# 12334zq/optical-flow-1

Measured on AMD Instinct MI355X. Metric: Mpix*warp-iters/s, TV-L1 1920x1080 5-scale, higher is better.
Workload: dtype f64; 1 GPU; tvl1flow 1920x1080 pair (synthetic P1), nscales=5 warps=5 tau=0.25 lambda=0.15 theta=0.3 zfactor=0.5 epsilon=0.01; one pair per step per GPU; workload_name=1080p, arithmetic_mode=tolerance, pairs_per_gpu=1040, pairs_in_flight_per_gpu=64, lockstep_group=16, streams_per_gpu=4, distinct_pairs=8

## Files before the change

optical-flow-1_amd/csrc/ofx_device.h:

```cpp
#pragma once

#include <hip/hip_runtime.h>

#define OFX_DEV __device__ __forceinline__

OFX_DEV double  ldw(const double *p) { return *p; }
OFX_DEV double  ldw(const float *p)  { return (double) *p; }
struct OfxRgb8 { unsigned char r, g, b; };
OFX_DEV unsigned gray8(unsigned r, unsigned g, unsigned b) { return (unsigned) (unsigned char) (.299 * r + .587 * g + .114 * b); }
OFX_DEV double  ldw(const unsigned char *p)  { return (double) *p; }
OFX_DEV double  ldw(const unsigned short *p) { return (double) *p; }
OFX_DEV double  ldw(const OfxRgb8 *p) { return (double) gray8(p->r, p->g, p->b); }
OFX_DEV double2 ldw2(const double2 *p) { return *p; }
OFX_DEV double2 ldw2(const float2 *p)  { float2 v = *p; return make_double2((double) v.x, (double) v.y); }
OFX_DEV double4 ldw4(const double4 *p) { return *p; }
OFX_DEV double4 ldw4(const float4 *p)
{
    float4 v = *p;
    return make_double4((double) v.x, (double) v.y, (double) v.z, (double) v.w);
}
OFX_DEV void stn(double *p, double v) { *p = v; }
OFX_DEV void stn(float *p, double v)  { *p = (float) v; }
OFX_DEV void stn2(double2 *p, double2 v) { *p = v; }
OFX_DEV void stn2(float2 *p, double2 v)  { *p = make_float2((float) v.x, (float) v.y); }
// ... 134 lines not shown
    const double r = __builtin_fma(-h, g, 0.5);
    g = __builtin_fma(g, r, g);
    double d = __builtin_fma(-g, g, x);
    h = __builtin_fma(h, r, h);
    g = __builtin_fma(d, h, g);
    d = __builtin_fma(-g, g, x);
    return __builtin_fma(d, h, g);
}
OFX_DEV double rcp_newton(double d)
{
    double r = __builtin_amdgcn_rcp(d);
    double e = __builtin_fma(-d, r, 1.0);
    r = __builtin_fma(r, e, r);
    e = __builtin_fma(-d, r, 1.0);
    return __builtin_fma(r, e, r);
}
OFX_DEV double div_unscaled(double n, double d)
{
    double r = __builtin_amdgcn_rcp(d);
    double e = __builtin_fma(-d, r, 1.0);
    r = __builtin_fma(r, e, r);
    e = __builtin_fma(-d, r, 1.0);
    r = __builtin_fma(r, e, r);
    const double q = n * r;
    const double rem = __builtin_fma(-d, q, n);
    return __builtin_fma(rem, r, q);
}
OFX_DEV double hypot_kernel_common(double ax, double ay)
{
    double h = sqrt_unscaled(ax * ax + ay * ay);
    double t1, t2;
    if (h <= 2.0 * ay) {
        const double delta = h - ay;
        t1 = ax * (2.0 * delta - ax);
        t2 = (delta - 2.0 * (ax - ay)) * delta;
    } else {
        const double delta = h - ax;
        t1 = 2.0 * delta * (ax - 2.0 * ay);
        t2 = (4.0 * delta - ay) * ay + delta * delta;
    }
    h -= div_unscaled(t1 + t2, 2.0 * h);
    return h;
}

OFX_DEV double hypot_ref(double x, double y)
{
    x = fabs(x);
    y = fabs(y);
    const double ax = x < y ? y : x;
    const double ay = x < y ? x : y;
    const double SCALE = 0x1p-600, LARGE = 0x1p+511, TINY = 0x1p-459, EPS = 0x1p-54;
#ifndef OFX_HYPOT_GENERAL_ONLY
    if (ax <= LARGE && ay >= 0x1p-383) {
        if (ax >= ay / EPS) return ax + ay;
        return hypot_kernel_common(ax, ay);
    }
#endif
    if (ax > LARGE) {
        if (ay <= ax * EPS) return ax + ay;
        return hypot_kernel(ax * SCALE, ay * SCALE) / SCALE;
    }
    if (ay < TINY) {
        if (ax >= ay / EPS) return ax + ay;
        return hypot_kernel(ax / SCALE, ay / SCALE) * SCALE;
    }
    if (ax >= ay / EPS) return ax + ay;
    return hypot_kernel(ax, ay);
}

struct BicubicTaps {
    int    col[4];
    int    row[4];
    double fx, fy;
    bool   out;
};

OFX_DEV int bc_clamp(int x, int n, bool &out)
{
    if (x < 0)  { out = true; return 0; }
    if (x >= n) { out = true; return n - 1; }
    return x;
}

OFX_DEV BicubicTaps bicubic_taps(double uu, double vv, int nx, int ny)
{
    BicubicTaps t;
    const int sx = (uu < 0) ? -1 : 1;
    const int sy = (vv < 0) ? -1 : 1;
    const int iu = (int) uu, iv = (int) vv;
    bool out = false;
    t.col[1] = bc_clamp(iu, nx, out);
    t.row[1] = bc_clamp(iv, ny, out);
    t.col[0] = bc_clamp(iu - sx, nx, out);
    t.row[0] = bc_clamp(iv - sx, ny, out);
    t.col[2] = bc_clamp(iu + sx, nx, out);
    t.row[2] = bc_clamp(iv + sy, ny, out);
    t.col[3] = bc_clamp(iu + 2 * sx, nx, out);
    t.row[3] = bc_clamp(iv + 2 * sy, ny, out);
    t.out = out;
    t.fx = uu - t.col[1];
    t.fy = vv - t.row[1];
    return t;
}

OFX_DEV double cubic_cell(double v0, double v1, double v2, double v3, double x)
{
    return v1 + 0.5 * x * (v2 - v0 + x * (2.0 * v0 - 5.0 * v1 + 4.0 * v2 - v3 + x * (3.0 * (v1 - v2) + v3 - v0)));
}

template <typename T>
OFX_DEV double bicubic_sample(const T *in, const BicubicTaps &t, int nx)
{
    double c[4];
#pragma unroll
    for (int k = 0; k < 4; k++) {
        const double v0 = ldw(in + (size_t) t.row[0] * nx + t.col[k]);
        const double v1 = ldw(in + (size_t) t.row[1] * nx + t.col[k]);
        const double v2 = ldw(in + (size_t) t.row[2] * nx + t.col[k]);
        const double v3 = ldw(in + (size_t) t.row[3] * nx + t.col[k]);
        c[k] = cubic_cell(v0, v1, v2, v3, t.fy);
    }
    return cubic_cell(c[0], c[1], c[2], c[3], t.fx);
}

template <typename V2, typename S>
OFX_DEV void bicubic_sample3(const V2 *__restrict__ pa, const S *__restrict__ pb, const BicubicTaps &t, int nx,
                             double &o0, double &o1, double &o2)
{
    const unsigned E = sizeof(S);
    const unsigned r0 = (unsigned) t.row[0] * nx * E, r1 = (unsigned) t.row[1] * nx * E;
    const unsigned r2 = (unsigned) t.row[2] * nx * E, r3 = (unsigned) t.row[3] * nx * E;
    double c0[4], c1[4], c2[4];
#pragma unroll
    for (int k = 0; k < 4; k++) {
        const unsigned ck = (unsigned) t.col[k] * E;
        const char *ba = reinterpret_cast<const char *>(pa), *bb = reinterpret_cast<const char *>(pb);
        const double2 a0 = ldw2(reinterpret_cast<const V2 *>(ba + 2 * (r0 + ck)));
        const double2 a1 = ldw2(reinterpret_cast<const V2 *>(ba + 2 * (r1 + ck)));
        const double2 a2 = ldw2(reinterpret_cast<const V2 *>(ba + 2 * (r2 + ck)));
        const double2 a3 = ldw2(reinterpret_cast<const V2 *>(ba + 2 * (r3 + ck)));
        const double b0 = ldw(reinterpret_cast<const S *>(bb + r0 + ck));
        const double b1 = ldw(reinterpret_cast<const S *>(bb + r1 + ck));
        const double b2 = ldw(reinterpret_cast<const S *>(bb + r2 + ck));
        const double b3 = ldw(reinterpret_cast<const S *>(bb + r3 + ck));
        c0[k] = cubic_cell(a0.x, a1.x, a2.x, a3.x, t.fy);
        c1[k] = cubic_cell(a0.y, a1.y, a2.y, a3.y, t.fy);
        c2[k] = cubic_cell(b0, b1, b2, b3, t.fy);
    }
    o0 = cubic_cell(c0[0], c0[1], c0[2], c0[3], t.fx);
    o1 = cubic_cell(c1[0], c1[1], c1[2], c1[3], t.fx);
    o2 = cubic_cell(c2[0], c2[1], c2[2], c2[3], t.fx);
}

OFX_DEV double div_backward(double ac, double al, double bc, double bu, bool lef, bool rig, bool top, bool bot)
{
    if (!lef && !rig) {
        const double dxv = ac - al;
        return top ? dxv + bc : (bot ? dxv - bu : dxv + (bc - bu));
    }
    if (lef) return top ? ac + bc : (bot ? ac - bu : ac + bc - bu);
    return top ? -al + bc : (bot ? -al - bu : -al + bc - bu);
}
```

optical-flow-1_amd/csrc/ofx_tvl1.hip:

```cpp
#include "ofx_ops.h"
#include "ofx_device.h"
#include "ofx_loop.h"
#include "ofx_pairs.h"

#include <chrono>
#include <cmath>
#include <type_traits>

#define TVL1_GRAD_IS_ZERO 1E-10
#define TVL1_PRESMOOTHING_SIGMA 0.8
#define STRIP_OUT 62

#ifdef OFX_NO_RFL
#define OFX_WAVE_UNIFORM(x) (x)
#else
#define OFX_WAVE_UNIFORM(x) __builtin_amdgcn_readfirstlane(x)
#endif
template <typename T> struct RowIn {
    double2 u, p1, p2, a;
    double r;
};

template <typename V> OFX_DEV const V *at(const V *base, unsigned byte_off)
{
// ... 782 lines not shown
            if (niter > max_iter - k0) niter = max_iter - k0;
            if (scribe) dev->cursor[(launch + 1) & 1][g] = k0 + niter;
        }
    }
    if (idle) return;
    const int step = check ? 1 : 0;
    if (N == 4 && niter >= 4) {
        if constexpr (N == 4)
            tvl1_iter3_march<T, NT, STRICT, 4, N>(Uin, P1in, P2in, A, R, hu.out, h1.out, h2.out, err, slot0, step, gw, nx, ny, y0, yend,
                                                  ys, yl, lef, rig, owner, off, so, up12, up22, cur, l_t, theta, taut, ring);
    } else if (niter >= 3)
        tvl1_iter3_march<T, NT, STRICT, 3, N>(Uin, P1in, P2in, A, R, hu.out, h1.out, h2.out, err, slot0, step, gw, nx, ny, y0, yend, ys,
                                              yl, lef, rig, owner, off, so, up12, up22, cur, l_t, theta, taut);
    else if (niter == 2)
        tvl1_iter3_march<T, NT, STRICT, 2, N>(Uin, P1in, P2in, A, R, hu.out, h1.out, h2.out, err, slot0, step, gw, nx, ny, y0, yend, ys,
                                              yl, lef, rig, owner, off, so, up12, up22, cur, l_t, theta, taut);
    else
        tvl1_iter3_march<T, NT, STRICT, 1, N>(Uin, P1in, P2in, A, R, hu.out, h1.out, h2.out, err, slot0, step, gw, nx, ny, y0, yend, ys,
                                              yl, lef, rig, owner, off, so, up12, up22, cur, l_t, theta, taut);
}

template <typename T, bool NT, bool STRICT>
__global__ __launch_bounds__(256) __attribute__((amdgpu_waves_per_eu(OFX_ITER3_WAVES, OFX_ITER3_WAVES))) void k_tvl1_iter3(
    Tri<typename Pix<T>::v2> Ut, Tri<typename Pix<T>::v2> P1t, Tri<typename Pix<T>::v2> P2t,
    const typename Pix<T>::v2 *__restrict__ Ag, const T *__restrict__ Rg, double *__restrict__ errg, int k0, int check, int slot0,
    int nx, int ny, int rows, int strips_x, int strips_pad, double l_t, double theta, double taut, double eps2, unsigned incode,
    unsigned runmask, unsigned long long nit, int err_stride, OfxLoopDev *dev, int launch, double afac1, double afac2, double afac3,
    int max_iter)
{
    tvl1_unit<T, NT, STRICT, 3>(Ut, P1t, P2t, Ag, Rg, errg, k0, check, slot0, nx, ny, rows, strips_x, strips_pad, l_t, theta, taut, eps2,
                                incode, runmask, nit, err_stride, dev, launch, afac1, afac2, afac3, max_iter, nullptr);
}

template <typename T, bool NT, bool STRICT>
__global__ __launch_bounds__(256) __attribute__((amdgpu_waves_per_eu(OFX_ITER3_WAVES, OFX_ITER3_WAVES))) void k_tvl1_iter4(
    Tri<typename Pix<T>::v2> Ut, Tri<typename Pix<T>::v2> P1t, Tri<typename Pix<T>::v2> P2t,
    const typename Pix<T>::v2 *__restrict__ Ag, const T *__restrict__ Rg, double *__restrict__ errg, int k0, int check, int slot0,
    int nx, int ny, int rows, int strips_x, int strips_pad, double l_t, double theta, double taut, double eps2, unsigned incode,
    unsigned runmask, unsigned long long nit, int err_stride, OfxLoopDev *dev, int launch, double afac1, double afac2, double afac3,
    int max_iter)
{
    __shared__ Tvl1Ring rings[4];
    tvl1_unit<T, NT, STRICT, 4>(Ut, P1t, P2t, Ag, Rg, errg, k0, check, slot0, nx, ny, rows, strips_x, strips_pad, l_t, theta, taut, eps2,
                                incode, runmask, nit, err_stride, dev, launch, afac1, afac2, afac3, max_iter, &rings[threadIdx.x >> 6]);
}

#define TILE_RH 16
template <typename T, bool STRICT, int K>
__global__ __launch_bounds__(64 * TILE_RH) void k_tvl1_tile(
    Tri<typename Pix<T>::v2> Ut, Tri<typename Pix<T>::v2> P1t, Tri<typename Pix<T>::v2> P2t,
    const typename Pix<T>::v2 *__restrict__ Ag, const T *__restrict__ Rg, double *__restrict__ errg, int k0, int check, int slot0,
    int nx, int ny, int tiles_x, double l_t, double theta, double taut, double eps2, unsigned incode, unsigned runmask,
    unsigned long long nit, int err_stride)
{
    using v2 = typename Pix<T>::v2;
    static_assert(K < 16, "4 bits of `nit` per pair");
    __shared__ double2 s_p[2][TILE_RH][64];
    __shared__ double2 s_u[2][TILE_RH][64];
    const int lane = threadIdx.x & 63, w = threadIdx.x >> 6;
    const int g = blockIdx.y;
    if (!((runmask >> g) & 1u)) return;
    const int niter = (int) ((nit >> (4 * g)) & 15ull);
    const size_t npix = (size_t) nx * ny;
    const TriSel<v2> hu = pick3(Ut, incode, g, npix), h1 = pick3(P1t, incode, g, npix), h2 = pick3(P2t, incode, g, npix);
    double *__restrict__ err = errg + (size_t) g * err_stride;
    double prev[K];
#pragma unroll
    for (int i = 0; i < K; i++) prev[i] = (check && k0 - i > 0) ? loop_fetch_prev(err, k0 - i) : 0.0;

    constexpr int OW = 64 - 2 * K, OH = TILE_RH - 2 * K;
    const int tx = blockIdx.x % tiles_x, ty = blockIdx.x / tiles_x;
    const int c = tx * OW - K + lane, y = ty * OH - K + w;
    const int cc = c < 0 ? 0 : (c > nx - 1 ? nx - 1 : c), yc = y < 0 ? 0 : (y > ny - 1 ? ny - 1 : y);
    const bool inside = (c >= 0) && (c < nx) && (y >= 0) && (y < ny);
    const bool owner = inside && lane >= K && lane < 64 - K && w >= K && w < TILE_RH - K;
    const bool lef = (c == 0), rig = (c == nx - 1), top = (y == 0), bot = (y == ny - 1);
    const size_t p = (size_t) yc * nx + cc;
    double2 u = ldw2(hu.in + p), p1 = ldw2(h1.in + p), p2 = ldw2(h2.in + p);
    const double2 a = ldw2(Ag + (size_t) g * npix + p);
    const double r = ldw(Rg + (size_t) g * npix + p);
    if (check) {
#pragma unroll
        for (int i = 0; i < K; i++)
            if (k0 - i > 0 && !(loop_error_from_sum(wave_allreduce_sum(prev[i]), nx * ny, OFX_CRIT_MEAN) > eps2)) return;
    }
    double acc[K];
#pragma unroll
    for (int it = 0; it < K; it++) {
        acc[it] = 0.0;
        if (it < niter) {
            s_p[it & 1][w][lane] = make_double2(p1.y, p2.y);
            __syncthreads();
            const double2 up = s_p[it & 1][w > 0 ? w - 1 : 0][lane];
            const double l11 = wave_shift_up(p1.x), l21 = wave_shift_up(p2.x);
            const double2 un = tvl1_primal<T, STRICT>(u, a, r, p1, p2, l11, l21, up.x, up.y, lef, rig, top, bot, l_t, theta);
            if (owner) acc[it] = TVL1_TOL64<T, STRICT> ? du2_fma(un, u)
                : (un.x - u.x) * (un.x - u.x) + (un.y - u.y) * (un.y - u.y);
            s_u[it & 1][w][lane] = un;
            __syncthreads();
            const double2 dn = s_u[it & 1][w < TILE_RH - 1 ? w + 1 : w][lane];
            const double r1 = wave_shift_down(un.x), r2 = wave_shift_down(un.y);
            double2 q1, q2;
            tvl1_dual<T, STRICT>(p1, p2, un, r1, r2, dn, rig, bot, taut, q1, q2);
            u = un;
            p1 = make_double2(rnd_to<T>(q1.x), rnd_to<T>(q1.y));
            p2 = make_double2(rnd_to<T>(q2.x), rnd_to<T>(q2.y));
        }
    }
    if (owner) {
        const size_t po = (size_t) y * nx + c;
        stn2(hu.out + po, u);
        stn2(h1.out + po, p1);
        stn2(h2.out + po, p2);
    }
#pragma unroll
    for (int it = 0; it < K; it++)
        if (it < niter) loop_accumulate(err, slot0 + (check ? it : 0), acc[it], blockIdx.x * TILE_RH + w);
}

#ifndef OFX_WARP_BX
#define OFX_WARP_BX 64
#define OFX_WARP_BY 4
#endif
template <typename T>
__global__ void k_tvl1_warp(const typename Pix<T>::v2 *__restrict__ pag, const T *__restrict__ pbg, const T *__restrict__ I0g,
                            Tri<typename Pix<T>::v2> Ut,
                            typename Pix<T>::v2 *__restrict__ Ag, T *__restrict__ Rg, int nx, int ny, unsigned curcode)
{
    const int j = blockIdx.x * OFX_WARP_BX + threadIdx.x;
    const int i = blockIdx.y * OFX_WARP_BY + threadIdx.y;
    if (j >= nx || i >= ny) return;
    const int g = blockIdx.z;
    const size_t goff = (size_t) g * nx * ny;
    const typename Pix<T>::v2 *__restrict__ pa = pag + goff;
    const T *__restrict__ pb = pbg + goff;
    const T *__restrict__ I0 = I0g + goff;
    const typename Pix<T>::v2 *__restrict__ U = pick3(Ut, curcode, g, (size_t) nx * ny).in;
    typename Pix<T>::v2 *__restrict__ A = Ag + goff;
    T *__restrict__ R = Rg + goff;
    const size_t p = (size_t) i * nx + j;
    const double2 u = ldw2(U + p);
    const BicubicTaps t = bicubic_taps(j + u.x, i + u.y, nx, ny);
    double I1w = 0.0, I1wx = 0.0, I1wy = 0.0;
    if (!t.out) {
        bicubic_sample3(pa, pb, t, nx, I1w, I1wx, I1wy);
        I1wx = rnd_to<T>(I1wx);
        I1wy = rnd_to<T>(I1wy);
    }
    stn2(A + p, make_double2(I1wx, I1wy));
    stn(R + p, (I1w - I1wx * u.x - I1wy * u.y - ldw(I0 + p)));
}

#ifndef WARP_TW
#define WARP_TW 48
#define WARP_TH 16
#endif
#ifndef WARP_BY
#define WARP_BY 8
#endif
#ifndef WARP_WAVES
#define WARP_WAVES 8
#endif
#define WARP_ATTR __attribute__((amdgpu_waves_per_eu(WARP_WAVES, WARP_WAVES)))
#define WARP_NT (32 * WARP_BY)
#define WARP_NW (WARP_NT / 64)
template <typename T>
__global__ __launch_bounds__(WARP_NT) WARP_ATTR void k_tvl1_warp_lds(
    const typename Pix<T>::v2 *__restrict__ pag, const T *__restrict__ pbg, const T *__restrict__ I0g,
    Tri<typename Pix<T>::v2> Ut, typename Pix<T>::v2 *__restrict__ Ag, T *__restrict__ Rg, int nx, int ny,
    unsigned curcode)
{
    __shared__ double2 s_a[WARP_TH * WARP_TW];
    __shared__ double s_b[WARP_TH * WARP_TW];
    __shared__ int s_box[WARP_NW][4];
    const int tid = threadIdx.y * 32 + threadIdx.x, wave = tid >> 6;
    const int j = blockIdx.x * 32 + threadIdx.x;
    const int i = blockIdx.y * WARP_BY + threadIdx.y;
    const bool inside = (j < nx) && (i < ny);
    const int g = blockIdx.z;
    const size_t goff = (size_t) g * nx * ny;
    const typename Pix<T>::v2 *__restrict__ pa = pag + goff;
    const T *__restrict__ pb = pbg + goff;
    const typename Pix<T>::v2 *__restrict__ U = pick3(Ut, curcode, g, (size_t) nx * ny).in;
    const size_t p = (size_t) (inside ? i : 0) * nx + (inside ? j : 0);
    double2 u = make_double2(0.0, 0.0);
    BicubicTaps t;
    t.out = true;
    if (inside) {
        u = ldw2(U + p);
        t = bicubic_taps(j + u.x, i + u.y, nx, ny);
    }
    const bool need = inside && !t.out;
    int xlo = need ? t.col[0] : 0x7fffffff, xhi = need ? t.col[3] : -1;
    int ylo = need ? t.row[0] : 0x7fffffff, yhi = need ? t.row[3] : -1;
#pragma unroll
    for (int m = 32; m >= 1; m >>= 1) {
        xlo = min(xlo, __shfl_xor(xlo, m, 64)); xhi = max(xhi, __shfl_xor(xhi, m, 64));
        ylo = min(ylo, __shfl_xor(ylo, m, 64)); yhi = max(yhi, __shfl_xor(yhi, m, 64));
    }
    if ((tid & 63) == 0) { s_box[wave][0] = xlo; s_box[wave][1] = xhi; s_box[wave][2] = ylo; s_box[wave][3] = yhi; }
    __syncthreads();
#pragma unroll
    for (int w = 0; w < WARP_NW; w++) {
        xlo = min(xlo, s_box[w][0]); xhi = max(xhi, s_box[w][1]);
        ylo = min(ylo, s_box[w][2]); yhi = max(yhi, s_box[w][3]);
    }
    const int W = xhi - xlo + 1, H = yhi - ylo + 1;
    const bool any = (xhi >= 0);
    const bool tile = any && W <= WARP_TW && H <= WARP_TH;
    if (tile) {
        for (int k = tid; k < W * H; k += WARP_NT) {
            const int r = k / W, c = k - r * W;
            const size_t src = (size_t) (ylo + r) * nx + (xlo + c);
            s_a[r * WARP_TW + c] = ldw2(pa + src);
            s_b[r * WARP_TW + c] = ldw(pb + src);
        }
        __syncthreads();
    }
    if (!inside) return;
    double I1w = 0.0, I1wx = 0.0, I1wy = 0.0;
    if (need) {
        if (tile) {
            const int cx = t.col[0] - xlo, cy = t.row[0] - ylo;
            double c0[4], c1[4], c2[4];
#pragma unroll
            for (int k = 0; k < 4; k++) {
                const int o = cy * WARP_TW + cx + k;
                const double2 a0 = s_a[o], a1 = s_a[o + WARP_TW], a2 = s_a[o + 2 * WARP_TW], a3 = s_a[o + 3 * WARP_TW];
                const double b0 = s_b[o], b1 = s_b[o + WARP_TW], b2 = s_b[o + 2 * WARP_TW], b3 = s_b[o + 3 * WARP_TW];
                c0[k] = cubic_cell(a0.x, a1.x, a2.x, a3.x, t.fy);
                c1[k] = cubic_cell(a0.y, a1.y, a2.y, a3.y, t.fy);
                c2[k] = cubic_cell(b0, b1, b2, b3, t.fy);
            }
            I1w = cubic_cell(c0[0], c0[1], c0[2], c0[3], t.fx);
            I1wx = cubic_cell(c1[0], c1[1], c1[2], c1[3], t.fx);
            I1wy = cubic_cell(c2[0], c2[1], c2[2], c2[3], t.fx);
        } else {
            bicubic_sample3(pa, pb, t, nx, I1w, I1wx, I1wy);
        }
        I1wx = rnd_to<T>(I1wx);
        I1wy = rnd_to<T>(I1wy);
    }
    stn2(Ag + goff + p, make_double2(I1wx, I1wy));
    stn(Rg + goff + p, (I1w - I1wx * u.x - I1wy * u.y - ldw(I0g + goff + p)));
}

template <typename T>
__global__ void k_tvl1_zoom_in_g(Tri<typename Pix<T>::v2> Ut, unsigned curcode, typename Pix<T>::v2 *__restrict__ Uout, int nx,
                                 int ny, int nxx, int nyy, double fx, double fy, double scale)
{
    const int j1 = blockIdx.x * 64 + threadIdx.x;
    const int i1 = blockIdx.y * 4 + threadIdx.y;
    if (j1 >= nxx || i1 >= nyy) return;
    const int g = blockIdx.z;
    const typename Pix<T>::v2 *__restrict__ U = pick3(Ut, curcode, g, (size_t) nx * ny).in;
    const double i2 = i1 / fy, j2 = j1 / fx;
    const BicubicTaps t = bicubic_taps(j2, i2, nx, ny);
    double c1[4], c2[4];
#pragma unroll
    for (int k = 0; k < 4; k++) {
        const double2 v0 = ldw2(U + (size_t) t.row[0] * nx + t.col[k]);
        const double2 v1 = ldw2(U + (size_t) t.row[1] * nx + t.col[k]);
        const double2 v2 = ldw2(U + (size_t) t.row[2] * nx + t.col[k]);
        const double2 v3 = ldw2(U + (size_t) t.row[3] * nx + t.col[k]);
        c1[k] = cubic_cell(v0.x, v1.x, v2.x, v3.x, t.fy);
        c2[k] = cubic_cell(v0.y, v1.y, v2.y, v3.y, t.fy);
    }
    double2 r;
    r.x = cubic_cell(c1[0], c1[1], c1[2], c1[3], t.fx) * scale;
    r.y = cubic_cell(c2[0], c2[1], c2[2], c2[3], t.fx) * scale;
    stn2(Uout + (size_t) g * nxx * nyy + (size_t) i1 * nxx + j1, r);
}

template <typename T>
__global__ void k_tvl1_to_flo_g(Tri<typename Pix<T>::v2> Ut, unsigned curcode, OfxGroupPtrs out, size_t n)
{
    const size_t i = (size_t) blockIdx.x * blockDim.x + threadIdx.x;
    if (i >= n) return;
    const int g = blockIdx.y;
    const double2 v = ldw2(pick3(Ut, curcode, g, n).in + i);
    ((float2 *) out.a[g])[i] = make_float2((float) v.x, (float) v.y);
}

template <typename T> struct Tvl1Level {
    using v2 = typename Pix<T>::v2;
    using v4 = typename Pix<T>::v4;
    int nx, ny, G;
    int shared;
    T  *I0, *I1;
    v2 *pa;
    T  *pb;
    v2 *U[3], *P1[3], *P2[3], *A;
    T  *R;
    unsigned cur;
    int last_n[OFX_MAX_GROUP];
    size_t n() const { return (size_t) nx * ny; }
    unsigned curidx(int g) const { return (cur >> (2 * g)) & 3u; }
    v2 *Ucur(int g) const { return U[curidx(g)] + (size_t) g * n(); }
    v2 *P1cur(int g) const { return P1[curidx(g)] + (size_t) g * n(); }
    v2 *P2cur(int g) const { return P2[curidx(g)] + (size_t) g * n(); }
    Tri<v2> Ut() const { return Tri<v2>{U[0], U[1], U[2]}; }
    Tri<v2> P1t() const { return Tri<v2>{P1[0], P1[1], P1[2]}; }
    Tri<v2> P2t() const { return Tri<v2>{P2[0], P2[1], P2[2]}; }
};

struct Tvl1Params {
    double tau, lambda, theta, epsilon;
    int warps, verbose, max_iter;
    bool fixed;
};

template <typename T> static int tvl1_level_alloc(ofx_ctx *ctx, Tvl1Level<T> &L, int nx, int ny, int G, bool images, int shared = 0)
{
    const size_t n = (size_t) nx * ny * G;
    L.nx = nx;
    L.ny = ny;
    L.G = G;
    L.shared = shared;
    L.cur = 0;
    for (int g = 0; g < OFX_MAX_GROUP; g++) L.last_n[g] = 0;
    L.I0 = L.I1 = nullptr;
    if (images) {
        OFX_TRY(ofx_alloc(ctx, n, &L.I0));
        if (!shared) OFX_TRY(ofx_alloc(ctx, n, &L.I1));
    }
    OFX_TRY(ofx_alloc(ctx, n, &L.pa));
    OFX_TRY(ofx_alloc(ctx, n, &L.pb));
    for (int h = 0; h < 3; h++) {
        OFX_TRY(ofx_alloc(ctx, n, &L.U[h]));
        OFX_TRY(ofx_alloc(ctx, n, &L.P1[h]));
        OFX_TRY(ofx_alloc(ctx, n, &L.P2[h]));
    }
    OFX_TRY(ofx_alloc(ctx, n, &L.A));
    OFX_TRY(ofx_alloc(ctx, n, &L.R));
    return OFX_OK;
}

static int tvl1_pick_rows(const ofx_ctx *ctx, int nx, int ny, int G)
{
    if (ctx->rows_per_wave > 0) return ctx->rows_per_wave;
    const long strips = (long) ofx_cdiv(nx, STRIP_OUT) * G;
    if (strips * ofx_cdiv(ny, 4) >= 2048) return 4;
    if (strips * ofx_cdiv(ny, 2) >= 1024) return 2;
    return 1;
}

static int tvl1_pick_rows2(const ofx_ctx *ctx, int nx, int ny, int G)
{
    if (ctx->rows_per_wave2 > 0) return ctx->rows_per_wave2;
    return ofx_pick_strip_rows(ofx_strip_model2(STRIP2_OUT, OFX_ITER2_WAVES), nx, ny, G, ctx->concurrency, ctx->rows_slots, INT_MAX);
}

static int tvl1_pick_chunk(const ofx_ctx *ctx, int nx, int ny, int G)
{
    if (ctx->chunk > 0) return ctx->chunk;
    const double est_us = fmax(5.0, (double) nx * ny * G * 120.0 / 4.0e6);
    int c = (int) (40.0 / est_us);
    return c < 4 ? 4 : (c > 50 ? 50 : c);
}

static int tvl1_pick_tile(const ofx_ctx *ctx, int nx, int ny, int G)
{
    if (!ctx->tile || !ctx->fuse2) return 0;
    const double lim = ctx->tile_max_px > 0 ? ctx->tile_max_px : 200000.0;
    if ((double) nx * ny * G > lim) return 0;
    return ctx->tile == 6 ? 6 : 4;
}

static int tvl1_pick_rows3(const ofx_ctx *ctx, int nx, int ny, int G, int N = 3)
{
    if (ctx->rows_per_wave3 > 0) return ctx->rows_per_wave3;
    {
        static const char *tab = getenv("OFX_ROWS3");
        for (const char *q = tab; q && *q;) {
            int lny = 0, r = 0;
            if (sscanf(q, "%d:%d", &lny, &r) == 2 && lny == ny && r > 0) return r;
            q = strchr(q, '/');
            if (q) q++;
        }
    }
    return ofx_pick_strip_rows(ofx_strip_model3(N, STRIP3_OUT, OFX_ITER3_WAVES), nx, ny, G, ctx->concurrency, ctx->rows_slots, ctx->rows3_max);
}

#ifndef TVL1_FUSE4_AUTO_PX
#define TVL1_FUSE4_AUTO_PX 2e6
#endif
template <typename T> struct Tvl1Launch {
    double l_t, taut, theta;
    bool strict;
    bool nt_stores;
    int err_stride;
    OfxUnitTable<3> units;
    Tvl1Launch(const ofx_ctx *ctx, const Tvl1Level<T> &L, const Tvl1Params &P)
        : l_t(P.lambda * P.theta), taut(P.tau / P.theta), theta(P.theta), strict(sizeof(T) == sizeof(double) && !ctx->relaxed_dual),
          nt_stores(ctx->nt_stores ? ctx->nt_stores == 1 : (double) L.nx * L.ny * L.G * 15.0 * sizeof(T) > 300e6),
          err_stride((P.max_iter + 1) * OFX_NSHARD), units(L.G, L.cur)
    {
    }
    template <class Fam> auto kernel(Fam fam) const -> decltype(fam(std::false_type{}, std::false_type{}))
    {
        if constexpr (sizeof(T) == sizeof(double)) {
            if (strict) return nt_stores ? fam(std::true_type{}, std::true_type{}) : fam(std::false_type{}, std::true_type{});
        }
        return nt_stores ? fam(std::true_type{}, std::false_type{}) : fam(std::false_type{}, std::false_type{});
    }
    void done(Tvl1Level<T> &L, const int *ran, const int *took_alt, const int *n_out) const
    {
        L.cur = units.result(ran, took_alt);
        for (int g = 0; g < L.G; g++) L.last_n[g] = n_out[g];
    }
};

template <typename T>
static int tvl1_run_iterations_tile(ofx_ctx *ctx, Tvl1Level<T> &L, const Tvl1Launch<T> &A, LoopSpec S, int K, int *n_out,
                                    double *err_out, float *ms_out, int *alt_out)
{
    const int nx = L.nx, ny = L.ny, G = L.G;
    const int OW = 64 - 2 * K, OH = TILE_RH - 2 * K;
    const int tiles_x = ofx_cdiv(nx, OW), tiles_y = ofx_cdiv(ny, OH);
    const dim3 grid((unsigned) (tiles_x * tiles_y), G), block(64 * TILE_RH);
    S.pairs = false;
    S.fuse = K;
    S.afac = 0.0;
    if (ctx->chunk <= 0) S.chunk = 6 * K;
    auto kern = A.kernel([&](auto, auto ST) { return K == 6 ? k_tvl1_tile<T, decltype(ST)::value, 6> : k_tvl1_tile<T, decltype(ST)::value, 4>; });
    auto go = [&](int k0, int check, int slot0, double thr, unsigned incode, unsigned runmask, unsigned long long nit) -> int {
        hipLaunchKernelGGL(kern, grid, block, 0, ctx->stream, L.Ut(), L.P1t(), L.P2t(), L.A, (const T *) L.R, ctx->d_err, k0, check,
                           slot0, nx, ny, tiles_x, A.l_t, A.theta, A.taut, thr, incode, runmask, nit, A.err_stride);
        OFX_LAUNCH_CHECK(ctx);
        return OFX_OK;
    };
    auto launch = [&](int k, int cnt, double thr) -> int { return go(k, 1, k, thr, A.units.code(k / K), A.units.all(), A.units.nit(cnt)); };
    auto redo = [&](const int *k_of) -> int {
        const auto r = A.units.redo(k_of, K);
        return go(0, 0, S.max_iter, -1.0, r.incode, r.runmask, r.nit);
    };
    OFX_TRY(ofx_run_loop_group(ctx, S, G, launch, redo, n_out, err_out, ms_out));
    int ran[OFX_MAX_GROUP];
    for (int g = 0; g < G; g++) {
        ran[g] = ofx_loop_units(n_out[g], K);
        if (alt_out) alt_out[g] = 0;
    }
    A.done(L, ran, nullptr, n_out);
    return OFX_OK;
}

template <typename T>
static int tvl1_run_iterations_tri(ofx_ctx *ctx, Tvl1Level<T> &L, const Tvl1Launch<T> &A, LoopSpec S, int N, int *n_out, double *err_out,
                                   float *ms_out, int *alt_out)
{
    const int nx = L.nx, ny = L.ny, G = L.G;
    const int rows = tvl1_pick_rows3(ctx, nx, ny, G, N);
    const int strips_x = ofx_cdiv(nx, STRIP3_OUT), strips_pad = ofx_cdiv(strips_x, 4) * 4;
    const dim3 grid((unsigned) (strips_pad / 4) * ofx_cdiv(ny, rows), G), block(256);
    S.pairs = false;
    S.fuse = N;
    S.afac = 0.0;
    const bool cursor = ctx->fuse3_cursor != 0 && !S.fixed;
    const double afac2 = ctx->fuse3_afac2 > 0 ? ctx->fuse3_afac2 : 1.5, afac1 = ctx->fuse3_afac1 > 0 ? ctx->fuse3_afac1 : 1.2;
    const double afac3 = ctx->fuse4_afac3 > 0 ? ctx->fuse4_afac3 : afac2;
    auto kern = A.kernel([&](auto NT, auto ST) {
        return N == 4 ? k_tvl1_iter4<T, decltype(NT)::value, decltype(ST)::value> : k_tvl1_iter3<T, decltype(NT)::value, decltype(ST)::value>;
    });
    auto go = [&](int k0, int check, int slot0, double thr, unsigned incode, unsigned runmask, unsigned long long nit, OfxLoopDev *dev,
                  int launch) -> int {
        hipLaunchKernelGGL(kern, grid, block, 0, ctx->stream, L.Ut(), L.P1t(), L.P2t(), L.A, (const T *) L.R, ctx->d_err, k0, check,
                           slot0, nx, ny, rows, strips_x, strips_pad, A.l_t, A.theta, A.taut, thr, incode, runmask, nit, A.err_stride, dev,
                           launch, afac1, afac2, afac3, S.max_iter);
        OFX_LAUNCH_CHECK(ctx);
        return OFX_OK;
    };
    auto rerun = [&](const OfxUnitTable<3>::Redo &r) -> int { return go(0, 0, S.max_iter, -1.0, r.incode, r.runmask, r.nit, nullptr, 0); };
    int ran[OFX_MAX_GROUP];
    int inside[OFX_MAX_GROUP];
    if (cursor) {
        auto launch = [&](int j, double thr) -> int {
            return go(0, 1, 0, thr, A.units.code((unsigned) j), A.units.all(), 0ull, reinterpret_cast<OfxLoopDev *>(ctx->d_state), j);
        };
        auto redo = [&](const int *n_of, const int *k0_of, const int *u_of) -> int { return rerun(A.units.redo(n_of, k0_of, u_of)); };
        const int upc = (S.chunk + N - 1) / N < 1 ? 1 : (S.chunk + N - 1) / N;
        OFX_TRY(ofx_run_loop_cursor(ctx, S, G, upc, N, launch, redo, n_out, err_out, ran, inside, ms_out));
        for (int g = 0; g < G; g++) ran[g]++;
    } else {
        auto launch = [&](int k, int cnt, double thr) -> int {
            return go(k, 1, k, thr, A.units.code((unsigned) (k / N)), A.units.all(), A.units.nit(cnt), nullptr, 0);
        };
        auto redo = [&](const int *k_of) -> int { return rerun(A.units.redo(k_of, N)); };
        OFX_TRY(ofx_run_loop_group(ctx, S, G, launch, redo, n_out, err_out, ms_out));
        for (int g = 0; g < G; g++) {
            ran[g] = ofx_loop_units(n_out[g], N);
            inside[g] = ofx_loop_inside(n_out[g], N, S.max_iter) ? 1 : 0;
        }
    }
    for (int g = 0; g < G && alt_out; g++) alt_out[g] = inside[g] ? 1 : 0;
    A.done(L, ran, nullptr, n_out);
    return OFX_OK;
}

template <typename T>
static int tvl1_run_iterations(ofx_ctx *ctx, Tvl1Level<T> &L, const Tvl1Params &P, int *n_out, double *err_out,
                               float *ms_out, int *alt_out = nullptr,
                               int *unit_out = nullptr)
{
    const int nx = L.nx, ny = L.ny, G = L.G;
    if ((long long) nx * ny >= (1LL << 27)) return ofx_fail(ctx, OFX_ERR_ARG, "tvl1: image larger than 2^27 pixels");
    const Tvl1Launch<T> A(ctx, L, P);
    const bool pairs = ctx->fuse2 != 0;
    const int rows = tvl1_pick_rows(ctx, nx, ny, G);
    const int strips_x = ofx_cdiv(nx, STRIP_OUT), strips_pad = ofx_cdiv(strips_x, 4) * 4;
    const unsigned gx1 = (unsigned) (strips_pad / 4) * ofx_cdiv(ny, rows);
    const dim3 block(256);
    const int rows2 = tvl1_pick_rows2(ctx, nx, ny, G);
    const int strips2_x = ofx_cdiv(nx, STRIP2_OUT), strips2_pad = ofx_cdiv(strips2_x, 4) * 4;
    const dim3 grid2((unsigned) (strips2_pad / 4) * ofx_cdiv(ny, rows2), G);
    LoopSpec S;
    S.max_iter = P.max_iter;
    S.size = nx * ny;
    S.thr = P.epsilon * P.epsilon;
    S.crit = OFX_CRIT_MEAN;
    S.chunk = tvl1_pick_chunk(ctx, nx, ny, G);
    S.fixed = P.fixed;
    S.pairs = pairs;
    const int tileK = tvl1_pick_tile(ctx, nx, ny, G);
    if (unit_out) *unit_out = tileK ? tileK : (pairs ? 2 : 1);
    if (tileK) return tvl1_run_iterations_tile<T>(ctx, L, A, S, tileK, n_out, err_out, ms_out, alt_out);
    {
        const double px = (double) nx * ny * G;
        const bool tri = ctx->fuse3 == 1 ? px >= ctx->fuse3_min_px
                                         : (ctx->fuse3 == 2 && !A.strict && (G >= 2 || ctx->concurrency > 1) &&
                                            px >= (ctx->fuse3_min_px > 0 ? ctx->fuse3_min_px : 5e5));
        const bool quad = ctx->fuse4 == 1 ? px >= ctx->fuse4_min_px
                                          : (ctx->fuse4 == 2 && tri && ctx->fuse3 == 2 &&
                                             px >= (ctx->fuse4_min_px > 0 ? ctx->fuse4_min_px : TVL1_FUSE4_AUTO_PX));
        if (pairs && (tri || quad)) {
            if (unit_out) *unit_out = quad ? 4 : 3;
            return tvl1_run_iterations_tri<T>(ctx, L, A, S, quad ? 4 : 3, n_out, err_out, ms_out, alt_out);
        }
    }
    const int F = pairs ? 2 : 1;
    const bool sa = pairs && !P.fixed && ctx->store_a != 0;
    S.afac = sa ? (ctx->store_a == 2 ? 1e300 : 1.5) : 0.0;
    unsigned amask0 = 0;
    if (sa)
        for (int g = 0; g < G; g++)
            if (ctx->store_a == 2 || (L.last_n[g] >= 1 && L.last_n[g] <= 2)) amask0 |= 1u << g;
    auto kern1 = A.kernel([](auto, auto ST) { return k_tvl1_iter<T, decltype(ST)::value>; });
    auto kern2 = A.kernel([](auto NT, auto ST) { return k_tvl1_iter2<T, decltype(NT)::value, decltype(ST)::value>; });
    auto single = [&](unsigned incode, unsigned runmask, int check, int slot, double thr) -> int {
        hipLaunchKernelGGL(kern1, dim3(gx1, G), block, 0, ctx->stream, L.Ut(), L.P1t(), L.P2t(), L.A, (const T *) L.R,
                           ctx->d_err, check, slot, nx, ny, rows, strips_x, strips_pad, A.l_t, A.theta, A.taut, thr, incode, runmask,
                           A.err_stride);
        OFX_LAUNCH_CHECK(ctx);
        return OFX_OK;
    };
    auto launch = [&](int k, int cnt, double thr) -> int {
        const unsigned incode = A.units.code((unsigned) (k / F));
        if (cnt == 1) return single(incode, A.units.all(), k, k, thr);
        const unsigned amask = k == 0 ? amask0 : 0u;
        hipLaunchKernelGGL(kern2, grid2, block, 0, ctx->stream, L.Ut(), L.P1t(), L.P2t(), L.A, (const T *) L.R, ctx->d_err, k, nx,
                           ny, rows2, strips2_x, strips2_pad, A.l_t, A.theta, A.taut, thr, incode, amask, S.afac, A.err_stride);
        OFX_LAUNCH_CHECK(ctx);
        return OFX_OK;
    };
    auto redo = [&](const int *k_of) -> int {
        const auto r = A.units.redo(k_of, F);
        return single(r.incode, r.runmask, 0, S.max_iter, -1.0);
    };
    int took_alt[OFX_MAX_GROUP], ran[OFX_MAX_GROUP];
    OFX_TRY(ofx_run_loop_group(ctx, S, G, launch, redo, n_out, err_out, ms_out, amask0, took_alt));
    for (int g = 0; g < G; g++) {
        ran[g] = ofx_loop_units(n_out[g], F);
        if (alt_out) alt_out[g] = ofx_loop_inside(n_out[g], F, S.max_iter) ? (took_alt[g] ? 2 : 1) : 0;
    }
    A.done(L, ran, took_alt, n_out);
    return OFX_OK;
}

template <typename T>
static int tvl1_single_scale_dev(ofx_ctx *ctx, Tvl1Level<T> &L, const Tvl1Params &P, int scale, ofx_stats *stats)
{
    const int nx = L.nx, ny = L.ny, G = L.G;
    const size_t n = L.n();
    const dim3 g2(ofx_cdiv(nx, OFX_WARP_BX), ofx_cdiv(ny, OFX_WARP_BY), G), b2(OFX_WARP_BX, OFX_WARP_BY);
    if (nx < 2 || ny < 2) return ofx_fail(ctx, OFX_ERR_ARG, "tvl1: level %dx%d too small", nx, ny);

    if (!L.shared) {
        OFX_TRY(op_grad_pack<T>(ctx, L.I1, L.pa, L.pb, nx, ny, G));
    } else {
        const size_t half = n * L.shared;
        OFX_TRY(op_grad_pack<T>(ctx, L.I0 + half, L.pa, L.pb, nx, ny, L.shared));
        OFX_TRY(op_grad_pack<T>(ctx, L.I0, L.pa + half, L.pb + half, nx, ny, L.shared));
    }
    for (int h = 0; h < 3; h++) {
        bool used = false;
        for (int g = 0; g < G; g++) used = used || (L.curidx(g) == (unsigned) h);
        if (!used) continue;
        OFX_TRY(op_fill2<T>(ctx, L.P1[h], n * G));
        OFX_TRY(op_fill2<T>(ctx, L.P2[h], n * G));
    }
    for (int g = 0; g < G; g++) L.last_n[g] = 0;

    for (int w = 0; w < P.warps; w++) {
        if (ctx->warp_lds)
            hipLaunchKernelGGL(k_tvl1_warp_lds<T>, dim3(ofx_cdiv(nx, 32), ofx_cdiv(ny, WARP_BY), G), dim3(32, WARP_BY), 0, ctx->stream, L.pa,
                               (const T *) L.pb, (const T *) L.I0, L.Ut(), L.A, L.R, nx, ny, L.cur);
        else
            hipLaunchKernelGGL(k_tvl1_warp<T>, g2, b2, 0, ctx->stream, L.pa, (const T *) L.pb, (const T *) L.I0, L.Ut(),
                               L.A, L.R, nx, ny, L.cur);
        OFX_LAUNCH_CHECK(ctx);
        int it[OFX_MAX_GROUP];
        double error[OFX_MAX_GROUP];
        float ms = 0.f;
        int odd[OFX_MAX_GROUP], unit = 0;
        OFX_TRY(tvl1_run_iterations<T>(ctx, L, P, it, error, ctx->profile ? &ms : nullptr, odd, &unit));
        if (P.verbose && G == 1) fprintf(stderr, "Warping: %d, Iterations: %d, Error: %f\n", w, it[0], error[0]);
        for (int g = 0; g < G; g++) {
            ofx_stats &S = stats[g];
            S.odd_stops += odd[g] != 0;
            S.odd_stops_stored += odd[g] == 2;
            if (scale < OFX_MAX_SCALES) {
                S.fused[scale] = unit;
                if (w < OFX_MAX_SOLVES) { S.iters[scale][w] = it[g]; S.error[scale][w] = error[g]; }
                S.iter_ms[scale] += ms;
                S.iter_launches[scale] += it[g];
            }
            S.work_pix_iters += (double) it[g] * nx * ny;
        }
        if (ctx->tvl1_median) {
            OfxMedianSlots M = {};
            for (int g = 0; g < G; g++) { M.in[g] = L.Ucur(g); M.out[g] = L.A + (size_t) g * n; }
            OFX_TRY(op_flow_median(ctx, (int) sizeof(T), ctx->tvl1_median, G, M, nx, ny));
            OFX_TRY(op_median_copy_back(ctx, (int) sizeof(T), G, M, n));
        }
    }
    return OFX_OK;
}

template <typename T>
static int tvl1_multiscale_dev(ofx_ctx *ctx, int G, const T *const *dI0, const T *const *dI1, int nxx, int nyy,
                               const Tvl1Params &P, int nscales, double zfactor, std::vector<Tvl1Level<T>> &lv,
                               ofx_stats *stats, int kind = -1, size_t pitch = 0,
                               int shared = 0,
                               const void *const *init = nullptr)
{
    const int Gp = shared ? shared : G;
    if (shared && G != 2 * shared) return ofx_fail(ctx, OFX_ERR_ARG, "tvl1: %d slots for %d bidirectional pairs", G, shared);
    if (P.warps < 1) return ofx_fail(ctx, OFX_ERR_ARG, "tvl1: warps=%d", P.warps);
    if (G < 1 || G > OFX_MAX_GROUP) return ofx_fail(ctx, OFX_ERR_ARG, "tvl1: group of %d pairs", G);

    using V2 = typename Pix<T>::v2;
    auto levels = [&](const std::vector<int> &nxs, const std::vector<int> &nys, T **lA, T **lB, V2 **U) -> int {
        lv.resize(nscales);
        for (int s = 0; s < nscales; s++) {
            OFX_TRY(tvl1_level_alloc<T>(ctx, lv[s], nxs[s], nys[s], G, true, shared));
            lA[s] = lv[s].I0;
            lB[s] = shared ? lv[s].I0 + (size_t) shared * lv[s].n() : lv[s].I1;
        }
        *U = lv[nscales - 1].U[0];
        return OFX_OK;
    };
    OFX_TRY(ofx_pyramid_head<T>(ctx, G, Gp, (const void *const *) dI0, (const void *const *) dI1, nxx, nyy, nscales, zfactor,
                                TVL1_PRESMOOTHING_SIGMA, P.warps, stats, kind, pitch, init, levels));

    for (int s = nscales - 1; s >= 0; s--) {
        if (P.verbose && G == 1) fprintf(stderr, "Scale %d: %dx%d\n", s, lv[s].nx, lv[s].ny);
        OFX_TRY(tvl1_single_scale_dev<T>(ctx, lv[s], P, s, stats));
        if (!s) break;
        lv[s - 1].cur = 0;
        {
            const int nxf = lv[s - 1].nx, nyf = lv[s - 1].ny;
            hipLaunchKernelGGL(k_tvl1_zoom_in_g<T>, dim3(ofx_cdiv(nxf, 64), ofx_cdiv(nyf, 4), G), dim3(64, 4), 0, ctx->stream,
                               lv[s].Ut(), lv[s].cur, lv[s - 1].U[0], lv[s].nx, lv[s].ny, nxf, nyf, (double) nxf / lv[s].nx,
                               (double) nyf / lv[s].ny, 1.0 / zfactor);
            OFX_LAUNCH_CHECK(ctx);
        }
    }
    return OFX_OK;
}

static Tvl1Params make_params(const ofx_ctx *ctx, double tau, double lambda, double theta, int warps,
                               double epsilon, int verbose)
{
    Tvl1Params P;
    P.tau = tau; P.lambda = lambda; P.theta = theta; P.epsilon = epsilon;
    P.warps = warps; P.verbose = verbose;
    P.max_iter = OFX_TVL1_MAX_ITERATIONS;
    P.fixed = ctx->fixed_work != 0;
    return P;
}

template <typename T>
static int tvl1_multiscale_host(ofx_ctx *ctx, const double *I0, const double *I1, double *u1, double *u2, int nx,
                                int ny, const Tvl1Params &P, int nscales, double zfactor)
{
    const size_t n = (size_t) nx * ny;
    T *dI0, *dI1;
    OFX_TRY(upload_plane<T>(ctx, I0, n, &dI0));
    OFX_TRY(upload_plane<T>(ctx, I1, n, &dI1));
    std::vector<Tvl1Level<T>> lv;
    const T *a = dI0, *b = dI1;
    OFX_TRY(tvl1_multiscale_dev<T>(ctx, 1, &a, &b, nx, ny, P, nscales, zfactor, lv, &ctx->stats));
    double *d1, *d2;
    OFX_TRY(ofx_alloc(ctx, n, &d1));
    OFX_TRY(ofx_alloc(ctx, n, &d2));
    OFX_TRY(op_deinterleave2<T>(ctx, lv[0].Ucur(0), d1, d2, n));
    OFX_HIP(ctx, hipMemcpyAsync(u1, d1, n * sizeof(double), hipMemcpyDeviceToHost, ctx->stream));
    OFX_HIP(ctx, hipMemcpyAsync(u2, d2, n * sizeof(double), hipMemcpyDeviceToHost, ctx->stream));
    OFX_HIP(ctx, hipStreamSynchronize(ctx->stream));
    return OFX_OK;
}

extern "C" int ofx_tvl1_multiscale(ofx_ctx *ctx, const double *I0, const double *I1, double *u1, double *u2, int nx,
                                   int ny, double tau, double lambda, double theta, int nscales, double zfactor,
                                   int warps, double epsilon, int verbose)
{
    OFX_ENTER(ctx);
    if (!I0 || !I1 || !u1 || !u2) return ofx_fail(ctx, OFX_ERR_ARG, "tvl1: NULL pointer");
    const double t0 = ofx_now_ms();
    const Tvl1Params P = make_params(ctx, tau, lambda, theta, warps, epsilon, verbose);
    int s = ctx->precision == OFX_F64
                ? tvl1_multiscale_host<double>(ctx, I0, I1, u1, u2, nx, ny, P, nscales, zfactor)
                : tvl1_multiscale_host<float>(ctx, I0, I1, u1, u2, nx, ny, P, nscales, zfactor);
    ctx->stats.total_ms = ofx_now_ms() - t0;
    return s;
}

template <typename T>
static int tvl1_group_devapi(ofx_ctx *ctx, int G, const void *const *dI0_in, const void *const *dI1_in, void *const *d_flo_in,
                             int nx, int ny, const Tvl1Params &P, int nscales, double zfactor, ofx_stats *stats,
                             const void *const *init_in = nullptr)
{
    const size_t n = (size_t) nx * ny;
    OFX_TRY(ofx_pitch_check(ctx, "tvl1", nx));
    OfxPairIO io;
    OFX_TRY(ofx_pairs_stage(ctx, G, dI0_in, dI1_in, init_in, d_flo_in, nx, ny, true, io));
    std::vector<Tvl1Level<T>> lv;
    OFX_TRY(tvl1_multiscale_dev<T>(ctx, G, (const T *const *) io.a, (const T *const *) io.b, nx, ny, P, nscales, zfactor, lv, stats,
                                   io.kind, io.pitch, 0, init_in ? io.init : nullptr));
    OfxGroupPtrs out;
    for (int g = 0; g < OFX_MAX_GROUP; g++) { out.a[g] = g < G ? io.flo[g] : nullptr; out.b[g] = nullptr; }
    hipLaunchKernelGGL(k_tvl1_to_flo_g<T>, dim3((unsigned) ((n + 255) / 256), G), dim3(256), 0, ctx->stream, lv[0].Ut(), lv[0].cur,
                       out, n);
    OFX_LAUNCH_CHECK(ctx);
    return ofx_pairs_unstage(ctx, G, d_flo_in, io, n);
}

extern "C" int ofx_tvl1_multiscale_dev(ofx_ctx *ctx, const void *dI0, const void *dI1, void *d_flo, int nx, int ny,
                                       double tau, double lambda, double theta, int nscales, double zfactor,
                                       int warps, double epsilon, int verbose)
{
    OFX_ENTER(ctx);
    if (!dI0 || !dI1 || !d_flo) return ofx_fail(ctx, OFX_ERR_ARG, "tvl1: NULL pointer");
    const double t0 = ofx_now_ms();
    const Tvl1Params P = make_params(ctx, tau, lambda, theta, warps, epsilon, verbose);
    int s = ctx->precision == OFX_F64
                ? tvl1_group_devapi<double>(ctx, 1, &dI0, &dI1, &d_flo, nx, ny, P, nscales, zfactor, &ctx->stats)
                : tvl1_group_devapi<float>(ctx, 1, &dI0, &dI1, &d_flo, nx, ny, P, nscales, zfactor, &ctx->stats);
    ctx->stats.total_ms = ofx_now_ms() - t0;
// ... 357 lines not shown
```

Baseline: 88180 Mpix*warp-iters/s.

## Compute image gradients on the fly in LDS warp kernel instead of precomputed packs

```diff
diff --git a/optical-flow-1_amd/csrc/ofx_device.h b/optical-flow-1_amd/csrc/ofx_device.h
--- a/optical-flow-1_amd/csrc/ofx_device.h
+++ b/optical-flow-1_amd/csrc/ofx_device.h
@@ -310,6 +310,58 @@
     o2 = cubic_cell(c2[0], c2[1], c2[2], c2[3], t.fx);
 }
 
+template <typename T, typename Cell>
+OFX_DEV void bicubic_window3(const Cell &cell, double fx, double fy, double &o0, double &o1, double &o2)
+{
+    {
+        double c0[4], c2[4];
+#pragma unroll
+        for (int k = 0; k < 4; k++) {
+            double m[6], gy[4];
+#pragma unroll
+            for (int a = 0; a < 6; a++) m[a] = cell(a, k + 1);
+#pragma unroll
+            for (int a = 0; a < 4; a++) gy[a] = rnd_to<T>(0.5 * (m[a + 2] - m[a]));
+            c0[k] = cubic_cell(m[1], m[2], m[3], m[4], fy);
+            c2[k] = cubic_cell(gy[0], gy[1], gy[2], gy[3], fy);
+            __builtin_amdgcn_sched_barrier(0);
+        }
+        o0 = cubic_cell(c0[0], c0[1], c0[2], c0[3], fx);
+        o2 = cubic_cell(c2[0], c2[1], c2[2], c2[3], fx);
+    }
+    __builtin_amdgcn_sched_barrier(0);
+    double c1[4];
+#pragma unroll
+    for (int h = 0; h < 2; h++) {
+        double l[4], r[4], gx[4];
+#pragma unroll
+        for (int a = 0; a < 4; a++) { l[a] = cell(a + 1, h); r[a] = cell(a + 1, h + 2); }
+#pragma unroll
+        for (int a = 0; a < 4; a++) gx[a] = rnd_to<T>(0.5 * (r[a] - l[a]));
+        c1[h] = cubic_cell(gx[0], gx[1], gx[2], gx[3], fy);
+        __builtin_amdgcn_sched_barrier(0);
+#pragma unroll
+        for (int a = 0; a < 4; a++) l[a] = cell(a + 1, h + 4);
+#pragma unroll
+        for (int a = 0; a < 4; a++) gx[a] = rnd_to<T>(0.5 * (l[a] - r[a]));
+        c1[h + 2] = cubic_cell(gx[0], gx[1], gx[2], gx[3], fy);
+        __builtin_amdgcn_sched_barrier(0);
+    }
+    o1 = cubic_cell(c1[0], c1[1], c1[2], c1[3], fx);
+}
+
+template <typename T>
+OFX_DEV void bicubic_sample3_image(const T *__restrict__ f, const BicubicTaps &t, int nx, int ny, double &o0, double &o1,
+                                   double &o2)
+{
+    const int x0 = t.col[0] - 1, y0 = t.row[0] - 1;
+    auto cell = [&](int r, int c) -> double {
+        const int y = min(max(y0 + r, 0), ny - 1), x = min(max(x0 + c, 0), nx - 1);
+        return ldw(f + (size_t) y * nx + x);
+    };
+    bicubic_window3<T>(cell, t.fx, t.fy, o0, o1, o2);
+}
+
 OFX_DEV double div_backward(double ac, double al, double bc, double bu, bool lef, bool rig, bool top, bool bot)
 {
     if (!lef && !rig) {
diff --git a/optical-flow-1_amd/csrc/ofx_tvl1.hip b/optical-flow-1_amd/csrc/ofx_tvl1.hip
--- a/optical-flow-1_amd/csrc/ofx_tvl1.hip
+++ b/optical-flow-1_amd/csrc/ofx_tvl1.hip
@@ -958,8 +958,8 @@
 }
 
 #ifndef WARP_TW
-#define WARP_TW 48
-#define WARP_TH 16
+#define WARP_TW 50
+#define WARP_TH 18
 #endif
 #ifndef WARP_BY
 #define WARP_BY 8
@@ -972,12 +972,10 @@
 #define WARP_NW (WARP_NT / 64)
 template <typename T>
 __global__ __launch_bounds__(WARP_NT) WARP_ATTR void k_tvl1_warp_lds(
-    const typename Pix<T>::v2 *__restrict__ pag, const T *__restrict__ pbg, const T *__restrict__ I0g,
-    Tri<typename Pix<T>::v2> Ut, typename Pix<T>::v2 *__restrict__ Ag, T *__restrict__ Rg, int nx, int ny,
-    unsigned curcode)
-{
-    __shared__ double2 s_a[WARP_TH * WARP_TW];
-    __shared__ double s_b[WARP_TH * WARP_TW];
+    const T *__restrict__ I1g, int shared, const T *__restrict__ I0g, Tri<typename Pix<T>::v2> Ut,
+    typename Pix<T>::v2 *__restrict__ Ag, T *__restrict__ Rg, int nx, int ny, unsigned curcode)
+{
+    __shared__ double s_f[WARP_TH * WARP_TW];
     __shared__ int s_box[WARP_NW][4];
     const int tid = threadIdx.y * 32 + threadIdx.x, wave = tid >> 6;
     const int j = blockIdx.x * 32 + threadIdx.x;
@@ -985,8 +983,7 @@
     const bool inside = (j < nx) && (i < ny);
     const int g = blockIdx.z;
     const size_t goff = (size_t) g * nx * ny;
-    const typename Pix<T>::v2 *__restrict__ pa = pag + goff;
-    const T *__restrict__ pb = pbg + goff;
+    const T *__restrict__ I1 = I1g + (size_t) (shared ? (g + shared) % (int) gridDim.z : g) * nx * ny;
     const typename Pix<T>::v2 *__restrict__ U = pick3(Ut, curcode, g, (size_t) nx * ny).in;
     const size_t p = (size_t) (inside ? i : 0) * nx + (inside ? j : 0);
     double2 u = make_double2(0.0, 0.0);
@@ -1011,38 +1008,27 @@
         xlo = min(xlo, s_box[w][0]); xhi = max(xhi, s_box[w][1]);
         ylo = min(ylo, s_box[w][2]); yhi = max(yhi, s_box[w][3]);
     }
-    const int W = xhi - xlo + 1, H = yhi - ylo + 1;
     const bool any = (xhi >= 0);
+    const int W = xhi - xlo + 3, H = yhi - ylo + 3;
     const bool tile = any && W <= WARP_TW && H <= WARP_TH;
     if (tile) {
-        for (int k = tid; k < W * H; k += WARP_NT) {
-            const int r = k / W, c = k - r * W;
-            const size_t src = (size_t) (ylo + r) * nx + (xlo + c);
-            s_a[r * WARP_TW + c] = ldw2(pa + src);
-            s_b[r * WARP_TW + c] = ldw(pb + src);
-        }
+        static_assert(WARP_TW <= 64, "a tile row is loaded by one wave");
+        const int c = tid & 63, x = min(max(xlo - 1 + c, 0), nx - 1);
+        if (c < W)
+            for (int r = wave; r < H; r += WARP_NW) {
+                const int y = min(max(ylo - 1 + r, 0), ny - 1);
+                s_f[r * WARP_TW + c] = ldw(I1 + (size_t) y * nx + x);
+            }
         __syncthreads();
     }
     if (!inside) return;
     double I1w = 0.0, I1wx = 0.0, I1wy = 0.0;
     if (need) {
         if (tile) {
-            const int cx = t.col[0] - xlo, cy = t.row[0] - ylo;
-            double c0[4], c1[4], c2[4];
-#pragma unroll
-            for (int k = 0; k < 4; k++) {
-                const int o = cy * WARP_TW + cx + k;
-                const double2 a0 = s_a[o], a1 = s_a[o + WARP_TW], a2 = s_a[o + 2 * WARP_TW], a3 = s_a[o + 3 * WARP_TW];
-                const double b0 = s_b[o], b1 = s_b[o + WARP_TW], b2 = s_b[o + 2 * WARP_TW], b3 = s_b[o + 3 * WARP_TW];
-                c0[k] = cubic_cell(a0.x, a1.x, a2.x, a3.x, t.fy);
-                c1[k] = cubic_cell(a0.y, a1.y, a2.y, a3.y, t.fy);
-                c2[k] = cubic_cell(b0, b1, b2, b3, t.fy);
-            }
-            I1w = cubic_cell(c0[0], c0[1], c0[2], c0[3], t.fx);
-            I1wx = cubic_cell(c1[0], c1[1], c1[2], c1[3], t.fx);
-            I1wy = cubic_cell(c2[0], c2[1], c2[2], c2[3], t.fx);
+            const double *__restrict__ s0 = s_f + (t.row[0] - ylo) * WARP_TW + (t.col[0] - xlo);
+            bicubic_window3<T>([&](int r, int c) -> double { return s0[r * WARP_TW + c]; }, t.fx, t.fy, I1w, I1wx, I1wy);
         } else {
-            bicubic_sample3(pa, pb, t, nx, I1w, I1wx, I1wy);
+            bicubic_sample3_image(I1, t, nx, ny, I1w, I1wx, I1wy);
         }
         I1wx = rnd_to<T>(I1wx);
         I1wy = rnd_to<T>(I1wy);
@@ -1130,8 +1116,12 @@
         OFX_TRY(ofx_alloc(ctx, n, &L.I0));
         if (!shared) OFX_TRY(ofx_alloc(ctx, n, &L.I1));
     }
-    OFX_TRY(ofx_alloc(ctx, n, &L.pa));
-    OFX_TRY(ofx_alloc(ctx, n, &L.pb));
+    L.pa = nullptr;
+    L.pb = nullptr;
+    if (!ctx->warp_lds) {
+        OFX_TRY(ofx_alloc(ctx, n, &L.pa));
+        OFX_TRY(ofx_alloc(ctx, n, &L.pb));
+    }
     for (int h = 0; h < 3; h++) {
         OFX_TRY(ofx_alloc(ctx, n, &L.U[h]));
         OFX_TRY(ofx_alloc(ctx, n, &L.P1[h]));
@@ -1390,7 +1380,8 @@
     const dim3 g2(ofx_cdiv(nx, OFX_WARP_BX), ofx_cdiv(ny, OFX_WARP_BY), G), b2(OFX_WARP_BX, OFX_WARP_BY);
     if (nx < 2 || ny < 2) return ofx_fail(ctx, OFX_ERR_ARG, "tvl1: level %dx%d too small", nx, ny);
 
-    if (!L.shared) {
+    if (ctx->warp_lds) {
+    } else if (!L.shared) {
         OFX_TRY(op_grad_pack<T>(ctx, L.I1, L.pa, L.pb, nx, ny, G));
     } else {
         const size_t half = n * L.shared;
@@ -1408,8 +1399,8 @@
 
     for (int w = 0; w < P.warps; w++) {
         if (ctx->warp_lds)
-            hipLaunchKernelGGL(k_tvl1_warp_lds<T>, dim3(ofx_cdiv(nx, 32), ofx_cdiv(ny, WARP_BY), G), dim3(32, WARP_BY), 0, ctx->stream, L.pa,
-                               (const T *) L.pb, (const T *) L.I0, L.Ut(), L.A, L.R, nx, ny, L.cur);
+            hipLaunchKernelGGL(k_tvl1_warp_lds<T>, dim3(ofx_cdiv(nx, 32), ofx_cdiv(ny, WARP_BY), G), dim3(32, WARP_BY), 0, ctx->stream,
+                               (const T *) (L.shared ? L.I0 : L.I1), L.shared, (const T *) L.I0, L.Ut(), L.A, L.R, nx, ny, L.cur);
         else
             hipLaunchKernelGGL(k_tvl1_warp<T>, g2, b2, 0, ctx->stream, L.pa, (const T *) L.pb, (const T *) L.I0, L.Ut(),
                                L.A, L.R, nx, ny, L.cur);
```

New measurement: 86330 Mpix*warp-iters/s. -2.1%, worse.
